# CederGroupHub/chgnet

Hardware: AMD Instinct MI355X
Metric: structures/s (energy+force+stress) on batched ~50-atom crystals (higher is better)
Workload: dtype f32

## Files before the change

### chgnet_amd/_lib.py

```python

from __future__ import annotations

import ctypes
import os

c_int_p = ctypes.POINTER(ctypes.c_int32)
c_float_p = ctypes.POINTER(ctypes.c_float)

TASK_BITS = {"e": 1, "f": 2, "s": 4, "m": 8}

EXPORTED_SYMBOLS = (
    "chg_abi_version", "chg_device_count", "chg_weights_required", "chg_engine_create", "chg_engine_destroy", "chg_last_error",
    "chg_batch_upload", "chg_batch_build", "chg_batch_build_predict", "chg_debug_fetch_i32", "chg_batch_update_geometry", "chg_batch_free", "chg_batch_device_bytes",
    "chg_predict", "chg_synchronize", "chg_batch_download", "chg_timer_start", "chg_timer_stop_ms",
    "chg_profile_enable", "chg_profile_reset", "chg_profile_count", "chg_profile_read",
    "chg_debug_fetch", "chg_test_rows_gemm", "chg_test_split_gemm",
    "chg_engine_set_memory_limit", "chg_engine_memory_info", "chg_batch_bytes_required",
    "chg_stream_copy", "chg_backward", "chg_engine_build_stats", "chg_engine_update_weights",
    "chg_engine_set_graph_search", "chg_engine_cell_stats",
    "chg_comm_unique_id", "chg_comm_create", "chg_comm_all_gather_f32", "chg_comm_all_reduce_sum_f32", "chg_comm_barrier",
    "chg_comm_destroy", "chg_comm_last_error",
    "chg_comm_all_gather_f32_device", "chg_comm_all_reduce_sum_f32_device", "chg_comm_reserve", "chg_comm_info",
    "chg_backward_allreduce", "chg_batch_all_gather_energy", "chg_engine_stream", "chg_engine_device",
    "chg_host_alloc", "chg_host_free",
    "chg_relax_create", "chg_relax_run", "chg_relax_download", "chg_relax_free", "chg_test_relax_step",
    "chg_md_create", "chg_md_run", "chg_md_download", "chg_md_free", "chg_test_md_step",
)


class ModelDesc(ctypes.Structure):
    _fields_ = [
        ("n_conv", ctypes.c_int32), ("cutoff_coeff", ctypes.c_int32), ("is_intensive", ctypes.c_int32),
        ("has_composition", ctypes.c_int32), ("atom_graph_cutoff", ctypes.c_float),
        ("bond_graph_cutoff", ctypes.c_float), ("n_weights", ctypes.c_int64),
        ("n_mlp_hidden", ctypes.c_int32), ("mlp_out_bias", ctypes.c_int32),
    ]


class BatchHost(ctypes.Structure):
# ... 118 lines not shown
    lib.chg_batch_update_geometry.argtypes = [vp, vp, c_float_p, c_float_p]
    lib.chg_batch_free.argtypes = [vp, vp]
    lib.chg_batch_device_bytes.argtypes = [vp]
    lib.chg_batch_device_bytes.restype = ctypes.c_int64
    lib.chg_predict.argtypes = [vp, vp, ctypes.c_uint32]
    lib.chg_synchronize.argtypes = [vp]
    lib.chg_backward.argtypes = [vp, vp, c_float_p, c_float_p, c_float_p, c_float_p, c_float_p]
    lib.chg_backward_allreduce.argtypes = [vp, vp, c_float_p, c_float_p, c_float_p, c_float_p, vp, c_float_p]
    lib.chg_batch_all_gather_energy.argtypes = [vp, vp, vp, ctypes.c_int64, c_float_p]
    lib.chg_engine_stream.argtypes = [vp]
    lib.chg_engine_stream.restype = ctypes.c_void_p
    lib.chg_engine_device.argtypes = [vp]
    lib.chg_engine_update_weights.argtypes = [vp, c_float_p]
    lib.chg_batch_download.argtypes = [vp, vp, ctypes.POINTER(OutHost)]
    lib.chg_timer_start.argtypes = [vp]
    lib.chg_timer_stop_ms.argtypes = [vp, c_float_p]
    lib.chg_stream_copy.argtypes = [vp, ctypes.c_int64, ctypes.c_int, c_float_p]
    lib.chg_profile_enable.argtypes = [vp, ctypes.c_int]
    lib.chg_profile_reset.argtypes = [vp]
    lib.chg_profile_count.argtypes = [vp]
    lib.chg_profile_read.argtypes = [vp, ctypes.c_int, ctypes.c_char_p, ctypes.c_int, ctypes.POINTER(ctypes.c_int64), ctypes.POINTER(ctypes.c_double)]
    lib.chg_debug_fetch.argtypes = [vp, vp, ctypes.c_char_p, c_float_p, ctypes.c_int64, ctypes.POINTER(ctypes.c_int64)]
    lib.chg_test_rows_gemm.argtypes = [vp, c_float_p, c_float_p, c_float_p, c_float_p, ctypes.c_int, ctypes.c_int, ctypes.c_int]
    lib.chg_test_split_gemm.argtypes = [vp, c_float_p, c_float_p, c_float_p, ctypes.c_int, ctypes.c_int, ctypes.c_int]
    dp = ctypes.POINTER(ctypes.c_double)
    lib.chg_relax_create.argtypes = [vp, ctypes.POINTER(StructsHost), ctypes.POINTER(RelaxParams), ctypes.POINTER(vp)]
    lib.chg_relax_run.argtypes = [vp, vp, ctypes.c_int32, c_int_p]
    lib.chg_relax_download.argtypes = [vp, vp, ctypes.POINTER(RelaxOutHost)]
    lib.chg_relax_free.argtypes = [vp, vp]
    lib.chg_test_relax_step.argtypes = [vp, ctypes.POINTER(RelaxParams), ctypes.c_int32, c_int_p, dp, dp, dp, c_int_p, c_float_p, c_float_p,
                                        c_float_p, c_float_p, dp, dp]
    lib.chg_md_create.argtypes = [vp, ctypes.POINTER(StructsHost), dp, dp, ctypes.POINTER(MdParams), ctypes.POINTER(vp)]
    lib.chg_md_run.argtypes = [vp, vp, ctypes.c_int32]
    lib.chg_md_download.argtypes = [vp, vp, ctypes.POINTER(MdOutHost)]
    lib.chg_md_free.argtypes = [vp, vp]
    lib.chg_test_md_step.argtypes = [vp, ctypes.POINTER(MdParams), ctypes.c_int32, c_int_p, ctypes.c_int32, dp, dp, dp, dp, dp, c_int_p,
                                     c_float_p, c_float_p, c_float_p, dp, dp]
    for name in EXPORTED_SYMBOLS:
        fn = getattr(lib, name)
        if fn.restype is ctypes.c_int and name not in ("chg_device_count", "chg_profile_count"):
            fn.restype = ctypes.c_int
    _LIB = lib
    return lib


def task_mask(task: str) -> int:
# ... 5 lines not shown
```

### chgnet_amd/csrc/engine.hip

```cpp

#include "engine_internal.h"
#include <cstring>

namespace chgh {

template <int UNROLL>
__global__ __launch_bounds__(256) void k_stream_copy(const f32x4* __restrict__ src, f32x4* __restrict__ dst, size_t n) {
  const size_t stride = (size_t)gridDim.x * blockDim.x;
  size_t i = (size_t)blockIdx.x * blockDim.x + threadIdx.x;
  for (; i + (UNROLL - 1) * stride < n; i += UNROLL * stride) {
    f32x4 v[UNROLL];
#pragma unroll
    for (int u = 0; u < UNROLL; ++u) v[u] = __builtin_nontemporal_load(src + i + u * stride);
#pragma unroll
    for (int u = 0; u < UNROLL; ++u) __builtin_nontemporal_store(v[u], dst + i + u * stride);
  }
  for (; i < n; i += stride) dst[i] = src[i];
}

template <bool NT>
__global__ __launch_bounds__(256) void k_stream_copy_seg(const f32x4* __restrict__ src, f32x4* __restrict__ dst, size_t n) {
  constexpr size_t SEG = 1024;
  const size_t nseg = n / SEG;
  for (size_t sgm = blockIdx.x; sgm < nseg; sgm += gridDim.x) {
// ... 526 lines not shown
  hipFree(a); hipFree(b);
  *ms_per_iter = best;
  return s;
}

int chg_test_rows_gemm(chg_engine* eng, const float* x, const float* wt, const float* bias, float* y, int rows, int k, int nout) {
  if (!eng || !x || !wt || !y || rows <= 0) return CHG_EINVAL;
  HIP_TRY(eng, hipSetDevice(eng->device));
  float *dx = nullptr, *dw = nullptr, *db = nullptr, *dy = nullptr;
  HIP_TRY(eng, hipMalloc(&dx, sizeof(float) * (size_t)rows * k));
  HIP_TRY(eng, hipMalloc(&dw, sizeof(float) * (size_t)nout * k));
  HIP_TRY(eng, hipMalloc(&db, sizeof(float) * (size_t)nout));
  HIP_TRY(eng, hipMalloc(&dy, sizeof(float) * (size_t)rows * nout));
  HIP_TRY(eng, hipMemcpy(dx, x, sizeof(float) * (size_t)rows * k, hipMemcpyHostToDevice));
  HIP_TRY(eng, hipMemcpy(dw, wt, sizeof(float) * (size_t)nout * k, hipMemcpyHostToDevice));
  if (bias) HIP_TRY(eng, hipMemcpy(db, bias, sizeof(float) * (size_t)nout, hipMemcpyHostToDevice));
  int s = rows_gemm(eng, "test_gemm", k, nout, dx, k, nullptr, dw, bias ? db : nullptr, nullptr, 0, dy, nout, nullptr, rows, 0);
  if (s == CHG_OK && hipStreamSynchronize(eng->stream) != hipSuccess) { eng->err = "test gemm failed"; s = CHG_EHIP; }
  if (s == CHG_OK) hipMemcpy(y, dy, sizeof(float) * (size_t)rows * nout, hipMemcpyDeviceToHost);
  hipFree(dx); hipFree(dw); hipFree(db); hipFree(dy);
  return s;
}

int chg_test_split_gemm(chg_engine* eng, const float* x, const float* w, float* y, int rows, int f, int mode) {
  if (!eng || !x || !w || !y || rows <= 0 || (f != D && f != 2 * D) || mode < 0 || mode > 3) return CHG_EINVAL;
  HIP_TRY(eng, hipSetDevice(eng->device));
  const int kin = (mode & 1) ? f : D, nout = (mode & 1) ? D : f;
  float *dx = nullptr, *dw = nullptr, *dy = nullptr;
  HIP_TRY(eng, hipMalloc(&dx, sizeof(float) * (size_t)rows * kin));
  HIP_TRY(eng, hipMalloc(&dw, sizeof(float) * (size_t)f * D));
  HIP_TRY(eng, hipMalloc(&dy, sizeof(float) * (size_t)rows * nout));
  HIP_TRY(eng, hipMemcpy(dx, x, sizeof(float) * (size_t)rows * kin, hipMemcpyHostToDevice));
  HIP_TRY(eng, hipMemcpy(dw, w, sizeof(float) * (size_t)f * D, hipMemcpyHostToDevice));
  hipStream_t st = eng->stream;
  switch (mode * 2 + (f == D ? 0 : 1)) {
    case 0: launch_test_split<0, D>(st, dx, dw, dy, rows); break;
    case 1: launch_test_split<0, 2 * D>(st, dx, dw, dy, rows); break;
    case 2: launch_test_split<1, D>(st, dx, dw, dy, rows); break;
    case 3: launch_test_split<1, 2 * D>(st, dx, dw, dy, rows); break;
    case 4: launch_test_split<2, D>(st, dx, dw, dy, rows); break;
    case 5: launch_test_split<2, 2 * D>(st, dx, dw, dy, rows); break;
    case 6: launch_test_split<3, D>(st, dx, dw, dy, rows); break;
    default: launch_test_split<3, 2 * D>(st, dx, dw, dy, rows); break;
  }
  int s = CHG_OK;
  if (hipGetLastError() != hipSuccess || hipStreamSynchronize(st) != hipSuccess) { eng->err = "chg_test_split_gemm failed"; s = CHG_EHIP; }
// ... 7 lines not shown
```

### chgnet_amd/csrc/engine_internal.h

```cpp
#pragma once

#include "chgnet_hip.h"

#include <hip/hip_runtime.h>

#include <algorithm>
#include <cmath>
#include <cstdint>
#include <cstdio>
#include <cstdlib>
#include <cstring>
#include <functional>
#include <map>
#include <mutex>
#include <string>
#include <unordered_map>
#include <vector>

#include "mfma_tile.h"
#include "mfma_split.h"
#include "kernels_conv.h"
#include "kernels_angle_w.h"
#include "kernels_angle_blk.h"
#include "kernels_embed.h"
// ... 221 lines not shown
template <class T>
int d2h(chg_engine* eng, T* dst, const T* src, size_t n) {
  if (n == 0 || !dst) return CHG_OK;
  HIP_TRY(eng, hipMemcpyAsync(dst, src, n * sizeof(T), hipMemcpyDeviceToHost, eng->stream));
  return CHG_OK;
}

template <class K>
int set_lds(chg_engine* eng, K kernel, size_t bytes) {
  HIP_TRY(eng, hipFuncSetAttribute(reinterpret_cast<const void*>(kernel), hipFuncAttributeMaxDynamicSharedMemorySize, (int)bytes));
  return CHG_OK;
}

size_t layout_weights(const float* base, int L, Weights& w);
int grid_for(int rows, int max_blocks, int block_rows = BLOCK_ROWS);
int tile_grid(chg_engine* eng, int rows, int block_rows = BLOCK_ROWS);
int rows_gemm(chg_engine* eng, const char* label, int K, int NOUT, const float* X, int ldx, const int* in_idx, const float* Wt,
              const float* bias, const float* resid, int ldr, float* Y, int ldy, const int* out_idx, int rows, int accumulate);
int rows_gemm_out2(chg_engine* eng, const char* label, const float* X, const int* in_idx, const float* Wt, const float* Wt2,
                   const float* bias, float* Y, int ldy, int rows);
int rows_gemm_in2(chg_engine* eng, const char* label, const float* X, int ldx, const float* Wt, const float* Wt2, float* Y,
                  const int* out_idx, int rows, int accumulate);
int zero(chg_engine* eng, void* p, size_t bytes);
int build_images(chg_engine* eng);
int predict_set_lds(chg_engine* eng);
int atomconv_q_table(chg_engine* eng, chg_batch* b, int l);
AtomConvArgs atomconv_args(chg_engine* eng, chg_batch* b, int l);
AngleArgs angle_args(chg_batch* b, int slot, const float* ang, const float* w_ang, const GatedW& g, float* out);
int angle_table_grads(chg_engine* eng, chg_batch* b, int slot, const float* w_bij_t, const float* w_ctr_t);
BondEmbedTArgs bond_embed_args(chg_engine* eng, chg_batch* b);
AngleEmbedTArgs angle_embed_args(chg_engine* eng, chg_batch* b);
int run_predict(chg_engine* eng, chg_batch* b, uint32_t task);
void carve(chg_batch* b, char* base, size_t& total);
int prepare_windows(chg_engine* eng, chg_batch* b);
inline long team_min_angles() {
  static const long v = [] { const char* e = std::getenv("CHGNET_TEAM_MIN_ANGLES"); return e ? std::atol(e) : 131072L; }();
  return v;
}
inline long blk_max_angles() {
  static const long v = [] { const char* e = std::getenv("CHGNET_BLK_MAX_ANGLES"); return e ? std::atol(e) : (1L << 22); }();
  return v;
}
inline size_t blk_tile_bound(size_t A, size_t Eb, size_t N) { return (A + 14 * Eb + 9 * N) / 16 + 1; }
inline int upload_blk_cap(size_t N, size_t A, size_t Eb) {
  return (A > 0 && N + 1 <= 8192 && (long)A <= blk_max_angles()) ? (int)blk_tile_bound(A, Eb, N) : 0;
}
// ... 28 lines not shown
```

### chgnet_amd/csrc/engine_predict.hip

```cpp
#include "engine_internal.h"

#include "kernels_geom.h"
#include "kernels_angle_fa.h"
#include "kernels_chain.h"

namespace chgh {


struct Cursor {
  const float* base;
  size_t pos = 0;
  const float* take(size_t n) {
    pos += (4 - pos % 4) % 4;
    const float* p = base + pos;
    pos += n;
    return p;
  }
};

void take_gated_tail(Cursor& c, GatedW& g, const float*& w2c_t, const float*& w2g_t) {
  g.w2c = c.take(D * D); g.b2c = c.take(D); g.w2g = c.take(D * D); g.b2g = c.take(D);
  w2c_t = c.take(D * D); w2g_t = c.take(D * D);
}
void take_ln(Cursor& c, GatedW& g) {
// ... 509 lines not shown
  a.ang0 = b->ang[0]; a.Gang = b->Gang; a.Gu = b->Gu;
  return a;
}

static int embed_grid_mult() {
  static const int m = [] { const char* e = std::getenv("CHGNET_EMBED_GRID_MULT"); return e ? std::atoi(e) : 2; }();
  return m;
}

struct ChainBuilder {
  ChainArgs a{};
  int max_rows = 0;
  ChainProb& add(int rows) {
    ChainProb& p = a.p[a.n++];
    p = ChainProb{};
    p.rows = rows;
    max_rows = std::max(max_rows, rows);
    return p;
  }
  static void term(ChainProb& p, const float* X, int ldx, const int* idx, const float* W, int K) { p.t[p.nterms++] = ChainTerm{X, idx, W, ldx, K}; }
  static void out(ChainProb& p, const float* W, const float* bias, float* Y, int ldy, int ncols) { p.o[p.nouts++] = ChainOut{W, bias, Y, ldy, ncols}; }
};
int launch_chain(chg_engine* eng, const char* label, ChainBuilder& cb) {
  int blocks = 0;
  for (int i = 0; i < cb.a.n; ++i) {
    ChainProb& p = cb.a.p[i];
    p.col_blocks = 0;
    for (int o = 0; o < p.nouts; ++o) p.col_blocks += p.o[o].ncols / D;
    p.serial_outs = (p.Y1 && p.Y1 == p.add) ? 1 : 0;
    if (p.serial_outs) {
      if (p.nouts > 1 || (p.nouts == 1 && p.o[0].ncols != D)) { eng->err = "launch_chain: an in-place problem takes one 64-column output"; return CHG_EINVAL; }
      p.col_blocks = 1;
    }
    p.col_blocks = std::max(1, p.col_blocks);
    blocks += p.col_blocks;
  }
  if (cb.max_rows <= 0 || blocks == 0) return CHG_OK;
  int row_blocks = 1;
  for (int i = 0; i < cb.a.n; ++i) {
    const int rows_per_wg = chain_tiles_per_wg(cb.a.p[i].nterms) * TILE_ROWS;
    row_blocks = std::max(row_blocks, (cb.a.p[i].rows + rows_per_wg - 1) / rows_per_wg);
  }
  LaunchScope ls(eng, label);
  hipLaunchKernelGGL(k_rows_chain, dim3(row_blocks, blocks), dim3(BLOCK), chain_lds(), eng->stream, cb.a);
  HIP_TRY(eng, hipGetLastError());
  return CHG_OK;
}

int forward_tiny(chg_engine* eng, chg_batch* b, bool want_grad, bool want_m) {
  const Weights& w = eng->w;
  const int L = b->L;
  for (int l = 0; l < L - 1; ++l) {
    TRY(atomconv_fwd_kernel(eng, b, l, want_grad));
    {
      ChainBuilder cb;
      ChainProb& p = cb.add(b->N);
      cb.term(p, b->agg_l[l], D, nullptr, w.ac[l].w_out, D);
      p.bias1 = w.ac[l].b_out; p.add = b->atom[l]; p.lda = D; p.Y1 = b->atom[l + 1]; p.ldy1 = D;
      cb.out(p, w.bc[l].w_ctr, w.bc[l].b1, b->Sl[l], 2 * D, 2 * D);
      cb.out(p, w.ac[l + 1].w_cn, w.ac[l + 1].b1, b->Pl[l + 1], 4 * D, 2 * D);
      cb.out(p, w.ac[l + 1].w_cn + 2 * D * D, nullptr, b->Pl[l + 1] + 2 * D, 4 * D, 2 * D);
      if (l < L - 2) cb.out(p, w.au[l].w_ctr, w.au[l].b1, b->Sl[L + l], 2 * D, 2 * D);
      if (l == 0) {
        ChainProb& q = cb.add(b->Eb);
        q.add = b->hbc[0]; q.lda = D;
        cb.out(q, w.bc[0].w_bij, nullptr, b->Rl[0], 4 * D, 2 * D);
        cb.out(q, w.bc[0].w_bij + 2 * D * D, nullptr, b->Rl[0] + 2 * D, 4 * D, 2 * D);
      }
      TRY(launch_chain(eng, "chain_A", cb));
// ... 105 lines not shown
      LaunchScope ls(eng, "embed_fwd");
      hipLaunchKernelGGL(k_embed_all<false>, dim3(ea.g_bond1 + ea.g_bond2 + ea.g_angle), dim3(BLOCK), bond_embed_lds(), st, ea);
    } else { LaunchScope ls(eng, "bond_embed_fwd");
      static const int o4 = [] { const char* e = std::getenv("CHGNET_EMBED_O4"); return e ? std::atoi(e) : 1; }();
      if (o4) hipLaunchKernelGGL((k_bond_embed_fwd_o4<1>), dim3(grid_for(b->Eu, o4 * 2 * eng->num_cus)), dim3(BLOCK), bond_embed_lds(), st, bond_embed_args(eng, b));
      else
      hipLaunchKernelGGL((k_bond_embed_t<false, false, 1>), dim3(grid_for(b->Eu, 2 * eng->num_cus)), dim3(BLOCK), bond_embed_lds(), st, bond_embed_args(eng, b));
      if (b->Eb > 0)
        hipLaunchKernelGGL((k_bond_embed_t<false, false, 2>), dim3(grid_for(b->Eb, 2 * eng->num_cus)), dim3(BLOCK), bond_embed_lds(), st, bond_embed_args(eng, b)); }
  }
  if (b->A > 0 && !(tiny && b->Ed > 0)) {
    LaunchScope ls(eng, "angle_embed_fwd");
    static const int o4 = [] { const char* e = std::getenv("CHGNET_EMBED_O4"); return e ? std::atoi(e) : 1; }();
    if (o4) hipLaunchKernelGGL((k_angle_embed_fwd_o4<0>), dim3(grid_for(b->A, o4 * embed_grid_mult() * eng->num_cus)), dim3(BLOCK), angle_embed_lds(), st, angle_embed_args(eng, b));
    else
    hipLaunchKernelGGL((k_angle_embed_t<false>), dim3(grid_for(b->A, embed_grid_mult() * eng->num_cus)), dim3(BLOCK), angle_embed_lds(), st, angle_embed_args(eng, b));
  }
  if (!tiny) { LaunchScope ls(eng, "atom_embed");
    hipLaunchKernelGGL(k_atom_embed, g1((int64_t)b->N * (D / 4)), dim3(256), 0, st, b->z, w.emb, b->atom[0], b->N); }
  HIP_TRY(eng, hipGetLastError());

  if (!tiny) TRY(zero(eng, b->zero1, zero_bytes));
  static const bool chain_on = [] { const char* e = std::getenv("CHGNET_TINY_CHAIN"); return !e || std::atoi(e) != 0; }();
  const bool chained = tiny && chain_on && fuse_gq() && L >= 2 && b->Ed > 0 && b->A > 0 && b->Eb > 0 && b->p_table_done == 0;
  if (chained) {
    TRY(forward_tiny(eng, b, want_grad, want_m));
  } else {
  for (int l = 0; l < L - 1; ++l) {
    TRY(atomconv_fwd(eng, b, l, want_grad));
    if (b->A > 0) {
      TRY(bondconv_fwd(eng, b, l));
      if (l < L - 2) TRY(angleupd_fwd(eng, b, l));
    }
  }
  if (want_m) {
    LaunchScope ls(eng, "magmom");
    hipLaunchKernelGGL(k_magmom, dim3(wave_grid(eng, b->N)), dim3(256), 0, st, b->atom[L - 1], w.site_w, w.site_b, b->magmom, b->N);
  }
  TRY(atomconv_fwd(eng, b, L - 1, want_grad));
  }

  {
    ReadoutArgs r{};
    r.atom = b->atom[L]; r.atom_owner = b->atom_owner; r.z = b->z; r.n_atoms = b->N;
    r.ln_g = w.ro_ln_g; r.ln_b = w.ro_ln_b; r.w0 = w.mlp_w0; r.b0 = w.mlp_b0; r.w1 = w.mlp_w1; r.b1 = w.mlp_b1;
    r.w2 = w.mlp_w2; r.b2 = w.mlp_b2; r.w3 = w.mlp_w3; r.b3 = w.mlp_b3; r.atomref = w.atomref;
    r.has_composition = eng->desc.has_composition; r.n_hidden = eng->desc.n_mlp_hidden;
    r.site_energy = b->site_energy; r.site_raw = b->site_raw; r.crystal_fea = b->crystal_fea;
// ... 256 lines not shown
  if ((s = set_lds(eng, k_angle_bwd_w<false>, angle_w_lds<false>()))) return s;
  if ((s = set_lds(eng, (k_angle_bwd_w<true, true>), angle_w_lds<true>()))) return s;
  if ((s = set_lds(eng, (k_angle_bwd_w<true, false, true>), angle_w_lds<true>()))) return s;
  if ((s = set_lds(eng, (k_angle_bwd_w<true, true, true>), angle_w_lds<true>()))) return s;
  if ((s = set_lds(eng, (k_angle_bwd_w<false, true>), angle_w_lds<false>()))) return s;
  if ((s = set_lds(eng, k_angle<true, false>, angle_lds<true>()))) return s;
  if ((s = set_lds(eng, k_angle<true, true>, (angle_lds<true, WAVES, true>())))) return s;
  if ((s = set_lds(eng, k_angle<false, true>, (angle_lds<false, WAVES, true>())))) return s;
  if ((s = set_lds(eng, k_angle<false, false, FWD_WAVES>, (angle_lds<false, FWD_WAVES>())))) return s;
#ifdef CHG_EXPERIMENTS
  if ((s = set_lds(eng, (k_angle<true, false, 4>), (size_t)100 << 10))) return s;
  if ((s = set_lds(eng, (k_angle<false, false, 4>), (size_t)100 << 10))) return s;
  if ((s = set_lds(eng, k_atomconv_fwd<4>, (size_t)100 << 10))) return s;
#endif
  if ((s = set_lds(eng, k_readout<false>, readout_lds()))) return s;
  if ((s = set_lds(eng, (k_bond_embed_t<false, false, 1>), bond_embed_lds()))) return s;
  if ((s = set_lds(eng, (k_bond_embed_t<false, false, 2>), bond_embed_lds()))) return s;
  if ((s = set_lds(eng, (k_bond_embed_t<true, false, 1>), bond_embed_lds()))) return s;
  if ((s = set_lds(eng, (k_bond_embed_t<true, false, 2>), bond_embed_lds()))) return s;
  if ((s = set_lds(eng, k_angle_embed_t<false>, angle_embed_lds()))) return s;
  if ((s = set_lds(eng, k_angle_embed_fwd_o4<0>, angle_embed_lds()))) return s;
  if ((s = set_lds(eng, k_bond_embed_fwd_o4<1>, bond_embed_lds()))) return s;
  if ((s = set_lds(eng, k_angle_embed_t<true>, angle_embed_lds()))) return s;
  if ((s = set_lds(eng, k_rows_chain, chain_lds()))) return s;
  if ((s = set_lds(eng, k_embed_all<false>, bond_embed_lds()))) return s;
  if ((s = set_lds(eng, k_embed_all<true>, bond_embed_lds()))) return s;
  return CHG_OK;
}


}
```

### chgnet_amd/csrc/kernels_chain.h

```cpp
#pragma once

#include "kernels_conv.h"

namespace chg {

constexpr int CHAIN_TERMS = 3, CHAIN_OUTS = 4, CHAIN_PROBS = 2;
struct ChainTerm {
  const float* X;
  const int* idx;
  const float* W;
  int ldx, K;
};
struct ChainOut {
  const float* W;
  const float* bias;
  float* Y;
  int ldy, ncols;
};
struct ChainProb {
  int rows, nterms, nouts, col_blocks;
  int serial_outs;
  ChainTerm t[CHAIN_TERMS];
  const float* bias1;
  const float* add;
  const int* add_idx;
  int lda;
  float* Y1;
  const int* y1_idx;
  int ldy1;
  ChainOut o[CHAIN_OUTS];
};
struct ChainArgs {
  ChainProb p[CHAIN_PROBS];
  int n;
};

__host__ __device__ constexpr int chain_tiles_per_wg(int nterms) { return nterms >= 2 ? 4 : WAVES; }
constexpr int CH_TS = D + PAD;
constexpr int CH_W1 = D * (2 * D + PAD);
constexpr size_t chain_lds() {
  return sizeof(float) * ((size_t)CHAIN_TERMS * CH_W1 + (size_t)D * (D + PAD) + D + D + (size_t)WAVES * TILE_ROWS * CH_TS);
}

struct ChainW { f32x4 v[4]; };
struct ChainX { f32x4 v[8]; };
__device__ __forceinline__ void chain_ws_issue(ChainW& r, const float* __restrict__ W, int K, int tid) {
  const int nchunks = (K / 32) * 4 * D;
#pragma unroll
  for (int q = 0; q < 2; ++q) {
    const int c = tid + q * BLOCK;
    if (c < nchunks) {
      const int f = c % D, g = (c / D) & 3, mk = c / (4 * D);
      const float* src = W + (size_t)f * K + 32 * mk + 4 * g;
      r.v[2 * q] = *reinterpret_cast<const f32x4*>(src);
      r.v[2 * q + 1] = *reinterpret_cast<const f32x4*>(src + 16);
    }
  }
}
__device__ __forceinline__ void chain_ws_commit(const ChainW& r, h16x8* img, int K, int tid) {
  const int nchunks = (K / 32) * 4 * D;
#pragma unroll
  for (int q = 0; q < 2; ++q) {
    const int c = tid + q * BLOCK;
    if (c < nchunks) {
      h16x8 hi, lo;
// ... 14 lines not shown
  }
}
template <int K>
__device__ __forceinline__ void chain_x_contract(f32x4 (&acc)[VT], const ChainX& r, const float* W1, float* T, int lane, int j, int g) {
  constexpr int LPR = K / 4, RPS = 64 / LPR, NV = TILE_ROWS / RPS, KT = K / 16;
  const int sub = lane / LPR, t = lane % LPR;
  f32x4 x[KT];
#pragma unroll
  for (int h = 0; h < K / D; ++h) {
    if ((t >> 4) == h) {
#pragma unroll
      for (int it = 0; it < NV; ++it) *reinterpret_cast<f32x4*>(T + (RPS * it + sub) * CH_TS + 4 * (t & 15)) = r.v[it];
    }
    __builtin_amdgcn_wave_barrier();
    f32x4 xh[VT];
    read_dl<VT>(T + j * CH_TS, g, xh);
#pragma unroll
    for (int f = 0; f < VT; ++f) x[VT * h + f] = xh[f];
    __builtin_amdgcn_wave_barrier();
  }
  gemm_split<KT, VT, true>(acc, reinterpret_cast<const h16x8*>(W1), D, x, j, g);
}

static __global__ __launch_bounds__(BLOCK) CHG_TWO_WAVES void k_rows_chain(ChainArgs a) {
  extern __shared__ __attribute__((aligned(16))) float smem[];
  float* W1 = smem;
  float* W2 = W1 + CHAIN_TERMS * CH_W1;
  float* b1s = W2 + D * (D + PAD);
  float* b2s = b1s + D;
  float* tiles = b2s + D;
  int y = blockIdx.y, pi = 0;
  for (; pi < a.n; ++pi) {
    if (y < a.p[pi].col_blocks) break;
    y -= a.p[pi].col_blocks;
  }
  if (pi >= a.n) return;
  const ChainProb& p = a.p[pi];
  const int cb = y;
  const int tpw = chain_tiles_per_wg(p.nterms);
  if ((int)blockIdx.x * tpw * TILE_ROWS >= p.rows) return;
  const int tid = threadIdx.x, wave = tid >> 6, lane = tid & 63, j = lane & 15, g = lane >> 4;
  const int row0 = (blockIdx.x * tpw + wave) * TILE_ROWS;
  const int nvalid = wave < tpw ? min(TILE_ROWS, p.rows - row0) : 0;
  const bool active = nvalid > 0;
  const int rr_ = active ? row0 + min(j, nvalid - 1) : 0;
  float* T = tiles + wave * TILE_ROWS * CH_TS;
  int in_row[CHAIN_TERMS];
#pragma unroll
  for (int t = 0; t < CHAIN_TERMS; ++t) in_row[t] = (t < p.nterms && p.t[t].idx) ? p.t[t].idx[rr_] : rr_;
  const int add_row = (p.add && p.add_idx) ? p.add_idx[rr_] : rr_;
  const int y1_row = (p.Y1 && p.y1_idx) ? p.y1_idx[rr_] : rr_;
  ChainW wr[CHAIN_TERMS], w2r;
#pragma unroll
  for (int t = 0; t < CHAIN_TERMS; ++t)
    if (t < p.nterms) chain_ws_issue(wr[t], p.t[t].W, p.t[t].K, tid);
  int lb = cb, oi = 0;
  for (; oi < p.nouts - 1; ++oi) {
    const int nb = p.o[oi].ncols >> 6;
    if (lb < nb) break;
    lb -= nb;
  }
  if (p.nouts) chain_ws_issue(w2r, p.o[oi].W + (size_t)lb * D * D, D, tid);
  float bias1 = 0.f, bias2 = 0.f;
  if (tid < D && p.bias1) bias1 = p.bias1[tid];
  if (p.nouts && tid < D && p.o[oi].bias) bias2 = p.o[oi].bias[lb * D + tid];
  ChainX xr[CHAIN_TERMS];
  const int sub4 = lane >> 4, t4 = lane & 15;
  f32x4 av[TILE_ROWS / 4];
  int orow[TILE_ROWS / 4];
  if (active) {
#pragma unroll
    for (int t = 0; t < CHAIN_TERMS; ++t)
      if (t < p.nterms) {
        if (p.t[t].K == D) chain_x_issue<D>(xr[t], p.t[t], in_row[t], lane);
        else chain_x_issue<2 * D>(xr[t], p.t[t], in_row[t], lane);
      }
#pragma unroll
    for (int it = 0; it < TILE_ROWS / 4; ++it) {
      const int rr = 4 * it + sub4;
      const int ra = __shfl(add_row, rr);
      orow[it] = __shfl(y1_row, rr);
      av[it] = zero4();
      if (p.add) av[it] = *reinterpret_cast<const f32x4*>(p.add + (size_t)ra * p.lda + 4 * t4);
    }
  }
  if (tid < D) { b1s[tid] = bias1; b2s[tid] = bias2; }
  if (p.nouts) chain_ws_commit(w2r, reinterpret_cast<h16x8*>(W2), D, tid);
#pragma unroll
  for (int t = 0; t < CHAIN_TERMS; ++t)
    if (t < p.nterms) chain_ws_commit(wr[t], reinterpret_cast<h16x8*>(W1 + t * CH_W1), p.t[t].K, tid);
  __syncthreads();
  if (!active) return;
  f32x4 acc[VT];
  read_dl<VT>(b1s, g, acc);
#pragma unroll
  for (int t = 0; t < CHAIN_TERMS; ++t)
    if (t < p.nterms) {
      if (p.t[t].K == D) chain_x_contract<D>(acc, xr[t], W1 + t * CH_W1, T, lane, j, g);
      else chain_x_contract<2 * D>(acc, xr[t], W1 + t * CH_W1, T, lane, j, g);
    }
  write_dl<VT>(T + j * CH_TS, g, acc);
  __builtin_amdgcn_wave_barrier();
#pragma unroll
  for (int it = 0; it < TILE_ROWS / 4; ++it) {
    av[it] += *reinterpret_cast<const f32x4*>(T + (4 * it + sub4) * CH_TS + 4 * t4);
    asm volatile("" : "+v"(av[it]));
  }
#pragma unroll
  for (int it = 0; it < TILE_ROWS / 4; ++it) {
    const int rr = 4 * it + sub4;
    *reinterpret_cast<f32x4*>(T + rr * CH_TS + 4 * t4) = av[it];
    if (p.Y1 && cb == 0 && rr < nvalid) *reinterpret_cast<f32x4*>(p.Y1 + (size_t)orow[it] * p.ldy1 + 4 * t4) = av[it];
  }
  if (p.nouts == 0) return;
  __builtin_amdgcn_wave_barrier();
  f32x4 x2[VT];
  read_dl<VT>(T + j * CH_TS, g, x2);
  __builtin_amdgcn_wave_barrier();
  const ChainOut& o = p.o[oi];
  f32x4 acc2[VT];
  read_dl<VT>(b2s, g, acc2);
  gemm_split<VT, VT, true>(acc2, reinterpret_cast<const h16x8*>(W2), D, x2, j, g);
  write_dl<VT>(T + j * CH_TS, g, acc2);
  __builtin_amdgcn_wave_barrier();
#pragma unroll
  for (int it = 0; it < TILE_ROWS / 4; ++it) {
    const int rr = 4 * it + sub4;
    if (rr < nvalid)
      *reinterpret_cast<f32x4*>(o.Y + (size_t)(row0 + rr) * o.ldy + lb * D + 4 * t4) = *reinterpret_cast<const f32x4*>(T + rr * CH_TS + 4 * t4);
  }
}

}
```

### chgnet_amd/engine.py

```python

from __future__ import annotations

import ctypes
import weakref

import numpy as np

from chgnet_amd import _lib
from chgnet_amd.graph.structure import atomic_numbers_of
from chgnet_amd.pack import D, PackedBatch, PackedWeights, _check_z, pack_batch


def _fp(a: np.ndarray):
    return a.ctypes.data_as(_lib.c_float_p)


def _ip(a: np.ndarray):
    return a.ctypes.data_as(_lib.c_int_p)


class PreparedStructures:

    __slots__ = ("n_struct", "z", "atom_off", "frac", "lattice")

# ... 291 lines not shown
            n, ms = ctypes.c_int64(), ctypes.c_double()
            self._check(self.lib.chg_profile_read(self.handle, i, buf, 64, ctypes.byref(n), ctypes.byref(ms)))
            out[buf.value.decode()] = (int(n.value), float(ms.value))
        return out

    def debug_fetch(self, batch: DeviceBatch, name: str, shape) -> np.ndarray:
        n = int(np.prod(shape))
        dst = np.empty(max(n, 1), np.float32)
        got = ctypes.c_int64()
        self._check(self.lib.chg_debug_fetch(self.handle, batch.handle, name.encode(), _fp(dst), n, ctypes.byref(got)))
        if got.value != n:
            raise RuntimeError(f"debug_fetch({name}): expected {n} floats, device buffer has {got.value}")
        return dst[:n].reshape(shape)

    def test_split_gemm(self, x: np.ndarray, w: np.ndarray, mode: int) -> np.ndarray:
        x = np.ascontiguousarray(x, np.float32)
        w = np.ascontiguousarray(w, np.float32)
        f = w.shape[0]
        assert w.shape[1] == 64 and x.shape[1] == (f if mode & 1 else 64)
        y = np.empty((x.shape[0], 64 if mode & 1 else f), np.float32)
        self._check(self.lib.chg_test_split_gemm(self.handle, _fp(x), _fp(w), _fp(y), x.shape[0], f, int(mode)))
        return y

    def test_rows_gemm(self, x: np.ndarray, wt: np.ndarray, bias: np.ndarray | None) -> np.ndarray:
        x = np.ascontiguousarray(x, np.float32)
        wt = np.ascontiguousarray(wt, np.float32)
        rows, k = x.shape
        nout = wt.shape[0]
        y = np.empty((rows, nout), np.float32)
        b = np.ascontiguousarray(bias, np.float32) if bias is not None else None
        self._check(self.lib.chg_test_rows_gemm(self.handle, _fp(x), _fp(wt), _fp(b) if b is not None else None, _fp(y), rows, k, nout))
        return y
```

### include/chgnet_hip.h

```cpp
#ifndef CHGNET_HIP_H
#define CHGNET_HIP_H

#include <stdint.h>

#ifdef __cplusplus
extern "C" {
#endif

typedef enum {
  CHG_OK = 0,
  CHG_EINVAL = -1,
  CHG_EHIP = -2,
  CHG_ENOMEM = -3,
  CHG_ENODEV = -4,
  CHG_EUNSUPPORTED = -5,
  CHG_ERANGE = -6
} chg_status;

enum {
  CHG_TASK_E = 1u,
  CHG_TASK_F = 2u,
  CHG_TASK_S = 4u,
  CHG_TASK_M = 8u
};
// ... 90 lines not shown
                 const float* force_cotangent, const float* stress_cotangent, float* grad_blob);
struct chg_comm;
int chg_backward_allreduce(chg_engine* eng, chg_batch* batch, const float* energy_cotangent, const float* magmom_cotangent,
                           const float* force_cotangent, const float* stress_cotangent, struct chg_comm* comm, float* grad_blob);
int chg_batch_all_gather_energy(chg_engine* eng, chg_batch* batch, struct chg_comm* comm, int64_t width, float* table);
void* chg_engine_stream(chg_engine* eng);
int chg_engine_device(chg_engine* eng);
int chg_engine_update_weights(chg_engine* eng, const float* weights_blob);
int chg_batch_download(chg_engine* eng, chg_batch* batch, const chg_out_host* out);

int chg_timer_start(chg_engine* eng);
int chg_timer_stop_ms(chg_engine* eng, float* elapsed_ms);

int chg_stream_copy(chg_engine* eng, int64_t bytes, int iters, float* ms_per_iter);

int chg_profile_enable(chg_engine* eng, int on);
int chg_profile_reset(chg_engine* eng);
int chg_profile_count(chg_engine* eng);
int chg_profile_read(chg_engine* eng, int i, char* label, int label_cap, int64_t* launches, double* total_ms);

int chg_debug_fetch(chg_engine* eng, chg_batch* batch, const char* name, float* dst, int64_t capacity, int64_t* n_written);

int chg_test_rows_gemm(chg_engine* eng, const float* x, const float* wt, const float* bias, float* y, int rows, int k, int nout);
int chg_test_split_gemm(chg_engine* eng, const float* x, const float* w, float* y, int rows, int f, int mode);

enum { CHG_RELAX_RUNNING = 0, CHG_RELAX_CONVERGED = 1, CHG_RELAX_MAX_STEPS = 2, CHG_RELAX_NONFINITE = 3 };
typedef struct chg_relax_params {
  double fmax;
  int32_t max_steps, relax_cell;
  double dt, maxstep, dtmax, finc, fdec, astart, fa;
  int32_t nmin;
  double exp_cell_factor;
  double r_atom, r_bond, numerical_tol;
  double stress_weight;
} chg_relax_params;
typedef struct chg_relax chg_relax;
typedef struct chg_relax_out_host {
  double* frac;
  double* lattice;
  float* energy;
  float* force;
  float* stress;
  float* magmom;
  int32_t* n_steps;
  int32_t* status;
} chg_relax_out_host;
// ... 72 lines not shown
```

Before: 38540.

## Make row-chain kernel persistent with multi-column weight staging and enable for all batches

The fused row-chain kernel becomes persistent: when the one-shot grid would exceed the CU count, each workgroup loops over row blocks and keeps several output-column weight blocks in LDS, reusing staged weights instead of reloading them per block. The kernel is templated on term count so LDS is sized to the actual number of terms, and the next tile's loads are issued early to overlap with compute. The chained forward path is no longer limited to tiny batches, so larger batches now take it as well. This risks lower occupancy from larger LDS use and less parallelism on big batches. A test entry point for the chain kernel is added.

```diff
diff --git a/chgnet_amd/_lib.py b/chgnet_amd/_lib.py
--- a/chgnet_amd/_lib.py
+++ b/chgnet_amd/_lib.py
@@ -14,7 +14,7 @@
     "chg_batch_upload", "chg_batch_build", "chg_batch_build_predict", "chg_debug_fetch_i32", "chg_batch_update_geometry", "chg_batch_free", "chg_batch_device_bytes",
     "chg_predict", "chg_synchronize", "chg_batch_download", "chg_timer_start", "chg_timer_stop_ms",
     "chg_profile_enable", "chg_profile_reset", "chg_profile_count", "chg_profile_read",
-    "chg_debug_fetch", "chg_test_rows_gemm", "chg_test_split_gemm",
+    "chg_debug_fetch", "chg_test_rows_gemm", "chg_test_rows_chain", "chg_test_split_gemm",
     "chg_engine_set_memory_limit", "chg_engine_memory_info", "chg_batch_bytes_required",
     "chg_stream_copy", "chg_backward", "chg_engine_build_stats", "chg_engine_update_weights",
     "chg_engine_set_graph_search", "chg_engine_cell_stats",
@@ -179,6 +179,7 @@
     lib.chg_profile_read.argtypes = [vp, ctypes.c_int, ctypes.c_char_p, ctypes.c_int, ctypes.POINTER(ctypes.c_int64), ctypes.POINTER(ctypes.c_double)]
     lib.chg_debug_fetch.argtypes = [vp, vp, ctypes.c_char_p, c_float_p, ctypes.c_int64, ctypes.POINTER(ctypes.c_int64)]
     lib.chg_test_rows_gemm.argtypes = [vp, c_float_p, c_float_p, c_float_p, c_float_p, ctypes.c_int, ctypes.c_int, ctypes.c_int]
+    lib.chg_test_rows_chain.argtypes = [vp, c_float_p, c_float_p, c_float_p, c_int_p, c_float_p, c_float_p, ctypes.c_int, ctypes.c_int]
     lib.chg_test_split_gemm.argtypes = [vp, c_float_p, c_float_p, c_float_p, ctypes.c_int, ctypes.c_int, ctypes.c_int]
     dp = ctypes.POINTER(ctypes.c_double)
     lib.chg_relax_create.argtypes = [vp, ctypes.POINTER(StructsHost), ctypes.POINTER(RelaxParams), ctypes.POINTER(vp)]
diff --git a/chgnet_amd/csrc/engine.hip b/chgnet_amd/csrc/engine.hip
--- a/chgnet_amd/csrc/engine.hip
+++ b/chgnet_amd/csrc/engine.hip
@@ -572,6 +572,34 @@
   return s;
 }
 
+int chg_test_rows_chain(chg_engine* eng, const float* x, const float* w, float* g, const int* idx, const float* wout, float* y, int rows, int n_g) {
+  if (!eng || !x || !w || !g || !idx || !wout || !y || rows <= 0 || n_g <= 0) return CHG_EINVAL;
+  for (int r = 0; r < rows; ++r)
+    if (idx[r] < 0 || idx[r] >= n_g) return CHG_EINVAL;
+  HIP_TRY(eng, hipSetDevice(eng->device));
+  float *dx = nullptr, *dw = nullptr, *dg = nullptr, *dwo = nullptr, *dy = nullptr;
+  int* di = nullptr;
+  HIP_TRY(eng, hipMalloc(&dx, sizeof(float) * (size_t)rows * 4 * D));
+  HIP_TRY(eng, hipMalloc(&dw, sizeof(float) * 4 * D * D));
+  HIP_TRY(eng, hipMalloc(&dg, sizeof(float) * (size_t)n_g * D));
+  HIP_TRY(eng, hipMalloc(&di, sizeof(int) * (size_t)rows));
+  HIP_TRY(eng, hipMalloc(&dwo, sizeof(float) * D * D));
+  HIP_TRY(eng, hipMalloc(&dy, sizeof(float) * (size_t)rows * D));
+  HIP_TRY(eng, hipMemcpy(dx, x, sizeof(float) * (size_t)rows * 4 * D, hipMemcpyHostToDevice));
+  HIP_TRY(eng, hipMemcpy(dw, w, sizeof(float) * 4 * D * D, hipMemcpyHostToDevice));
+  HIP_TRY(eng, hipMemcpy(dg, g, sizeof(float) * (size_t)n_g * D, hipMemcpyHostToDevice));
+  HIP_TRY(eng, hipMemcpy(di, idx, sizeof(int) * (size_t)rows, hipMemcpyHostToDevice));
+  HIP_TRY(eng, hipMemcpy(dwo, wout, sizeof(float) * D * D, hipMemcpyHostToDevice));
+  int s = test_rows_chain(eng, dx, dw, dg, di, dwo, dy, rows);
+  if (s == CHG_OK && hipStreamSynchronize(eng->stream) != hipSuccess) { eng->err = "test chain failed"; s = CHG_EHIP; }
+  if (s == CHG_OK) {
+    hipMemcpy(g, dg, sizeof(float) * (size_t)n_g * D, hipMemcpyDeviceToHost);
+    hipMemcpy(y, dy, sizeof(float) * (size_t)rows * D, hipMemcpyDeviceToHost);
+  }
+  hipFree(dx); hipFree(dw); hipFree(dg); hipFree(di); hipFree(dwo); hipFree(dy);
+  return s;
+}
+
 int chg_test_split_gemm(chg_engine* eng, const float* x, const float* w, float* y, int rows, int f, int mode) {
   if (!eng || !x || !w || !y || rows <= 0 || (f != D && f != 2 * D) || mode < 0 || mode > 3) return CHG_EINVAL;
   HIP_TRY(eng, hipSetDevice(eng->device));
diff --git a/chgnet_amd/csrc/engine_internal.h b/chgnet_amd/csrc/engine_internal.h
--- a/chgnet_amd/csrc/engine_internal.h
+++ b/chgnet_amd/csrc/engine_internal.h
@@ -267,6 +267,7 @@
 int rows_gemm_in2(chg_engine* eng, const char* label, const float* X, int ldx, const float* Wt, const float* Wt2, float* Y,
                   const int* out_idx, int rows, int accumulate);
 int zero(chg_engine* eng, void* p, size_t bytes);
+int test_rows_chain(chg_engine* eng, const float* X, const float* W, float* G, const int* idx, const float* Wout, float* Y, int rows);
 int build_images(chg_engine* eng);
 int predict_set_lds(chg_engine* eng);
 int atomconv_q_table(chg_engine* eng, chg_batch* b, int l);
diff --git a/chgnet_amd/csrc/engine_predict.hip b/chgnet_amd/csrc/engine_predict.hip
--- a/chgnet_amd/csrc/engine_predict.hip
+++ b/chgnet_amd/csrc/engine_predict.hip
@@ -555,29 +555,70 @@
   static void out(ChainProb& p, const float* W, const float* bias, float* Y, int ldy, int ncols) { p.o[p.nouts++] = ChainOut{W, bias, Y, ldy, ncols}; }
 };
 int launch_chain(chg_engine* eng, const char* label, ChainBuilder& cb) {
-  int blocks = 0;
-  for (int i = 0; i < cb.a.n; ++i) {
-    ChainProb& p = cb.a.p[i];
+  ChainArgs& A = cb.a;
+  A.nt1 = 1;
+  int one_shot_wgs = 0, max_row_blocks = 1;
+  for (int i = 0; i < A.n; ++i) {
+    ChainProb& p = A.p[i];
+    A.nt1 = std::max(A.nt1, p.nterms);
     p.col_blocks = 0;
     for (int o = 0; o < p.nouts; ++o) p.col_blocks += p.o[o].ncols / D;
     p.serial_outs = (p.Y1 && p.Y1 == p.add) ? 1 : 0;
-    if (p.serial_outs) {
-      if (p.nouts > 1 || (p.nouts == 1 && p.o[0].ncols != D)) { eng->err = "launch_chain: an in-place problem takes one 64-column output"; return CHG_EINVAL; }
-      p.col_blocks = 1;
+    if (p.serial_outs && (p.nouts > 1 || (p.nouts == 1 && p.o[0].ncols != D))) {
+      eng->err = "launch_chain: an in-place problem takes one 64-column output";
+      return CHG_EINVAL;
     }
     p.col_blocks = std::max(1, p.col_blocks);
-    blocks += p.col_blocks;
-  }
-  if (cb.max_rows <= 0 || blocks == 0) return CHG_OK;
-  int row_blocks = 1;
-  for (int i = 0; i < cb.a.n; ++i) {
-    const int rows_per_wg = chain_tiles_per_wg(cb.a.p[i].nterms) * TILE_ROWS;
-    row_blocks = std::max(row_blocks, (cb.a.p[i].rows + rows_per_wg - 1) / rows_per_wg);
+    p.tpw = chain_tiles_per_wg(p.nterms);
+    p.cpw = 1;
+    const int rows_per_wg = p.tpw * TILE_ROWS;
+    const int row_blocks = (p.rows + rows_per_wg - 1) / rows_per_wg;
+    max_row_blocks = std::max(max_row_blocks, row_blocks);
+    one_shot_wgs += row_blocks * p.col_blocks;
+  }
+  if (cb.max_rows <= 0) return CHG_OK;
+  int gx = max_row_blocks, gy = 0, cpw_max = 1;
+  if (one_shot_wgs <= eng->num_cus) {
+    for (int i = 0; i < A.n; ++i) { A.p[i].wgs = gx; gy += A.p[i].col_blocks; }
+  } else {
+    const size_t fixed = chain_lds_floats(A.nt1, 0), cap = chain_lds() / sizeof(float);
+    const int fit = std::max(1, (int)((cap - fixed) / (CH_W2 + D)));
+    long work = 0;
+    int rbs[CHAIN_PROBS];
+    for (int i = 0; i < A.n; ++i) {
+      ChainProb& p = A.p[i];
+      p.tpw = WAVES;
+      const int groups = (p.col_blocks + fit - 1) / fit;
+      p.cpw = (p.col_blocks + groups - 1) / groups;
+      p.col_blocks = groups;
+      cpw_max = std::max(cpw_max, p.cpw);
+      rbs[i] = (p.rows + WAVES * TILE_ROWS - 1) / (WAVES * TILE_ROWS);
+      work += (long)rbs[i] * groups;
+    }
+    gx = 1;
+    for (int i = 0; i < A.n; ++i) {
+      ChainProb& p = A.p[i];
+      p.wgs = (int)std::max<long>(1, std::min<long>(rbs[i], (long)eng->num_cus * rbs[i] / std::max<long>(1, work)));
+      gx = std::max(gx, p.wgs);
+      gy += p.col_blocks;
+    }
   }
   LaunchScope ls(eng, label);
-  hipLaunchKernelGGL(k_rows_chain, dim3(row_blocks, blocks), dim3(BLOCK), chain_lds(), eng->stream, cb.a);
+  const size_t lds = sizeof(float) * chain_lds_floats(A.nt1, cpw_max);
+  if (A.nt1 == 1) hipLaunchKernelGGL(k_rows_chain<1>, dim3(gx, gy), dim3(BLOCK), lds, eng->stream, A);
+  else hipLaunchKernelGGL(k_rows_chain<CHAIN_TERMS>, dim3(gx, gy), dim3(BLOCK), lds, eng->stream, A);
   HIP_TRY(eng, hipGetLastError());
   return CHG_OK;
+}
+
+int test_rows_chain(chg_engine* eng, const float* X, const float* W, float* G, const int* idx, const float* Wout, float* Y, int rows) {
+  ChainBuilder cb;
+  ChainProb& p = cb.add(rows);
+  cb.term(p, X, 4 * D, nullptr, W, 2 * D);
+  cb.term(p, X + 2 * D, 4 * D, nullptr, W + 2 * D * D, 2 * D);
+  p.add = G; p.add_idx = idx; p.lda = D; p.Y1 = G; p.y1_idx = idx; p.ldy1 = D;
+  cb.out(p, Wout, nullptr, Y, D, D);
+  return launch_chain(eng, "test_chain", cb);
 }
 
 int forward_tiny(chg_engine* eng, chg_batch* b, bool want_grad, bool want_m) {
@@ -729,8 +770,9 @@
 
   if (!tiny) TRY(zero(eng, b->zero1, zero_bytes));
   static const bool chain_on = [] { const char* e = std::getenv("CHGNET_TINY_CHAIN"); return !e || std::atoi(e) != 0; }();
-  const bool chained = tiny && chain_on && fuse_gq() && L >= 2 && b->Ed > 0 && b->A > 0 && b->Eb > 0 && b->p_table_done == 0;
+  const bool chained = chain_on && fuse_gq() && L >= 2 && b->Ed > 0 && b->A > 0 && b->Eb > 0;
   if (chained) {
+    TRY(atomconv_tables(eng, b, 0));
     TRY(forward_tiny(eng, b, want_grad, want_m));
   } else {
   for (int l = 0; l < L - 1; ++l) {
@@ -1033,7 +1075,8 @@
   if ((s = set_lds(eng, k_angle_embed_fwd_o4<0>, angle_embed_lds()))) return s;
   if ((s = set_lds(eng, k_bond_embed_fwd_o4<1>, bond_embed_lds()))) return s;
   if ((s = set_lds(eng, k_angle_embed_t<true>, angle_embed_lds()))) return s;
-  if ((s = set_lds(eng, k_rows_chain, chain_lds()))) return s;
+  if ((s = set_lds(eng, k_rows_chain<1>, chain_lds()))) return s;
+  if ((s = set_lds(eng, k_rows_chain<CHAIN_TERMS>, chain_lds()))) return s;
   if ((s = set_lds(eng, k_embed_all<false>, bond_embed_lds()))) return s;
   if ((s = set_lds(eng, k_embed_all<true>, bond_embed_lds()))) return s;
   return CHG_OK;
diff --git a/chgnet_amd/csrc/kernels_chain.h b/chgnet_amd/csrc/kernels_chain.h
--- a/chgnet_amd/csrc/kernels_chain.h
+++ b/chgnet_amd/csrc/kernels_chain.h
@@ -20,6 +20,9 @@
 struct ChainProb {
   int rows, nterms, nouts, col_blocks;
   int serial_outs;
+  int tpw;
+  int cpw;
+  int wgs;
   ChainTerm t[CHAIN_TERMS];
   const float* bias1;
   const float* add;
@@ -33,14 +36,17 @@
 struct ChainArgs {
   ChainProb p[CHAIN_PROBS];
   int n;
+  int nt1;
 };
 
 __host__ __device__ constexpr int chain_tiles_per_wg(int nterms) { return nterms >= 2 ? 4 : WAVES; }
 constexpr int CH_TS = D + PAD;
 constexpr int CH_W1 = D * (2 * D + PAD);
-constexpr size_t chain_lds() {
-  return sizeof(float) * ((size_t)CHAIN_TERMS * CH_W1 + (size_t)D * (D + PAD) + D + D + (size_t)WAVES * TILE_ROWS * CH_TS);
-}
+constexpr int CH_W2 = D * (D + PAD);
+__host__ __device__ constexpr size_t chain_lds_floats(int nt1, int cpw) {
+  return (size_t)nt1 * CH_W1 + (size_t)cpw * (CH_W2 + D) + D + (size_t)WAVES * TILE_ROWS * CH_TS;
+}
+constexpr size_t chain_lds() { return sizeof(float) * chain_lds_floats(CHAIN_TERMS, 1); }
 
 struct ChainW { f32x4 v[4]; };
 struct ChainX { f32x4 v[8]; };
@@ -101,13 +107,49 @@
   gemm_split<KT, VT, true>(acc, reinterpret_cast<const h16x8*>(W1), D, x, j, g);
 }
 
-static __global__ __launch_bounds__(BLOCK) CHG_TWO_WAVES void k_rows_chain(ChainArgs a) {
+__device__ __forceinline__ void chain_block(const ChainProb& p, int gb, int& oi, int& lb) {
+  lb = gb; oi = 0;
+  for (; oi < p.nouts - 1; ++oi) {
+    const int nb = p.o[oi].ncols >> 6;
+    if (lb < nb) break;
+    lb -= nb;
+  }
+}
+
+template <int NT>
+struct ChainTile {
+  ChainX xr[NT];
+  f32x4 av[TILE_ROWS / 4];
+  int orow[TILE_ROWS / 4];
+};
+template <int NT>
+__device__ __forceinline__ void chain_tile_issue(ChainTile<NT>& c, const ChainProb& p, int row0, int nvalid, int lane) {
+  const int j = lane & 15, sub4 = lane >> 4, t4 = lane & 15;
+  const int rr_ = row0 + min(j, nvalid - 1);
+  int in_row[NT];
+#pragma unroll
+  for (int t = 0; t < NT; ++t) in_row[t] = (t < p.nterms && p.t[t].idx) ? p.t[t].idx[rr_] : rr_;
+  const int add_row = (p.add && p.add_idx) ? p.add_idx[rr_] : rr_;
+  const int y1_row = (p.Y1 && p.y1_idx) ? p.y1_idx[rr_] : rr_;
+#pragma unroll
+  for (int t = 0; t < NT; ++t)
+    if (t < p.nterms) {
+      if (p.t[t].K == D) chain_x_issue<D>(c.xr[t], p.t[t], in_row[t], lane);
+      else chain_x_issue<2 * D>(c.xr[t], p.t[t], in_row[t], lane);
+    }
+#pragma unroll
+  for (int it = 0; it < TILE_ROWS / 4; ++it) {
+    const int rr = 4 * it + sub4;
+    const int ra = __shfl(add_row, rr);
+    c.orow[it] = __shfl(y1_row, rr);
+    c.av[it] = zero4();
+    if (p.add) c.av[it] = *reinterpret_cast<const f32x4*>(p.add + (size_t)ra * p.lda + 4 * t4);
+  }
+}
+
+template <int NT>
+__global__ __launch_bounds__(BLOCK) CHG_TWO_WAVES void k_rows_chain(ChainArgs a) {
   extern __shared__ __attribute__((aligned(16))) float smem[];
-  float* W1 = smem;
-  float* W2 = W1 + CHAIN_TERMS * CH_W1;
-  float* b1s = W2 + D * (D + PAD);
-  float* b2s = b1s + D;
-  float* tiles = b2s + D;
   int y = blockIdx.y, pi = 0;
   for (; pi < a.n; ++pi) {
     if (y < a.p[pi].col_blocks) break;
@@ -115,99 +157,104 @@
   }
   if (pi >= a.n) return;
   const ChainProb& p = a.p[pi];
-  const int cb = y;
-  const int tpw = chain_tiles_per_wg(p.nterms);
-  if ((int)blockIdx.x * tpw * TILE_ROWS >= p.rows) return;
+  const int cg = y;
+  const int tpw = p.tpw;
+  if ((int)blockIdx.x >= p.wgs || (int)blockIdx.x * tpw * TILE_ROWS >= p.rows) return;
+  float* W1 = smem;
+  float* W2 = W1 + a.nt1 * CH_W1;
+  float* b2s = W2 + p.cpw * CH_W2;
+  float* b1s = b2s + p.cpw * D;
+  float* tiles = b1s + D;
   const int tid = threadIdx.x, wave = tid >> 6, lane = tid & 63, j = lane & 15, g = lane >> 4;
-  const int row0 = (blockIdx.x * tpw + wave) * TILE_ROWS;
-  const int nvalid = wave < tpw ? min(TILE_ROWS, p.rows - row0) : 0;
-  const bool active = nvalid > 0;
-  const int rr_ = active ? row0 + min(j, nvalid - 1) : 0;
+  const int sub4 = lane >> 4, t4 = lane & 15;
   float* T = tiles + wave * TILE_ROWS * CH_TS;
-  int in_row[CHAIN_TERMS];
-#pragma unroll
-  for (int t = 0; t < CHAIN_TERMS; ++t) in_row[t] = (t < p.nterms && p.t[t].idx) ? p.t[t].idx[rr_] : rr_;
-  const int add_row = (p.add && p.add_idx) ? p.add_idx[rr_] : rr_;
-  const int y1_row = (p.Y1 && p.y1_idx) ? p.y1_idx[rr_] : rr_;
-  ChainW wr[CHAIN_TERMS], w2r;
-#pragma unroll
-  for (int t = 0; t < CHAIN_TERMS; ++t)
+  int tot_blocks = 0;
+  for (int o = 0; o < p.nouts; ++o) tot_blocks += p.o[o].ncols >> 6;
+  const int blk0 = cg * p.cpw, nb = max(0, min(p.cpw, tot_blocks - blk0));
+  int rb = blockIdx.x;
+  int row0 = (rb * tpw + wave) * TILE_ROWS;
+  int nvalid = wave < tpw ? min(TILE_ROWS, p.rows - row0) : 0;
+  ChainW wr[NT], w2r;
+#pragma unroll
+  for (int t = 0; t < NT; ++t)
     if (t < p.nterms) chain_ws_issue(wr[t], p.t[t].W, p.t[t].K, tid);
-  int lb = cb, oi = 0;
-  for (; oi < p.nouts - 1; ++oi) {
-    const int nb = p.o[oi].ncols >> 6;
-    if (lb < nb) break;
-    lb -= nb;
-  }
-  if (p.nouts) chain_ws_issue(w2r, p.o[oi].W + (size_t)lb * D * D, D, tid);
+  int oi = 0, lb = 0;
+  if (nb) {
+    chain_block(p, blk0, oi, lb);
+    chain_ws_issue(w2r, p.o[oi].W + (size_t)lb * D * D, D, tid);
+  }
   float bias1 = 0.f, bias2 = 0.f;
   if (tid < D && p.bias1) bias1 = p.bias1[tid];
-  if (p.nouts && tid < D && p.o[oi].bias) bias2 = p.o[oi].bias[lb * D + tid];
-  ChainX xr[CHAIN_TERMS];
-  const int sub4 = lane >> 4, t4 = lane & 15;
-  f32x4 av[TILE_ROWS / 4];
-  int orow[TILE_ROWS / 4];
-  if (active) {
-#pragma unroll
-    for (int t = 0; t < CHAIN_TERMS; ++t)
+  if (nb && tid < D && p.o[oi].bias) bias2 = p.o[oi].bias[lb * D + tid];
+  ChainTile<NT> c;
+  if (nvalid > 0) chain_tile_issue(c, p, row0, nvalid, lane);
+  if (tid < D) { b1s[tid] = bias1; b2s[tid] = bias2; }
+  if (nb) chain_ws_commit(w2r, reinterpret_cast<h16x8*>(W2), D, tid);
+#pragma unroll
+  for (int t = 0; t < NT; ++t)
+    if (t < p.nterms) chain_ws_commit(wr[t], reinterpret_cast<h16x8*>(W1 + t * CH_W1), p.t[t].K, tid);
+  for (int k = 1; k < nb; ++k) {
+    chain_block(p, blk0 + k, oi, lb);
+    chain_ws_issue(w2r, p.o[oi].W + (size_t)lb * D * D, D, tid);
+    bias2 = (tid < D && p.o[oi].bias) ? p.o[oi].bias[lb * D + tid] : 0.f;
+    if (tid < D) b2s[k * D + tid] = bias2;
+    chain_ws_commit(w2r, reinterpret_cast<h16x8*>(W2 + k * CH_W2), D, tid);
+  }
+  __syncthreads();
+  while (nvalid > 0) {
+    f32x4 acc[VT];
+    read_dl<VT>(b1s, g, acc);
+#pragma unroll
+    for (int t = 0; t < NT; ++t)
       if (t < p.nterms) {
-        if (p.t[t].K == D) chain_x_issue<D>(xr[t], p.t[t], in_row[t], lane);
-        else chain_x_issue<2 * D>(xr[t], p.t[t], in_row[t], lane);
+        if (p.t[t].K == D) chain_x_contract<D>(acc, c.xr[t], W1 + t * CH_W1, T, lane, j, g);
+        else chain_x_contract<2 * D>(acc, c.xr[t], W1 + t * CH_W1, T, lane, j, g);
       }
+    write_dl<VT>(T + j * CH_TS, g, acc);
+    __builtin_amdgcn_wave_barrier();
+#pragma unroll
+    for (int it = 0; it < TILE_ROWS / 4; ++it) {
+      c.av[it] += *reinterpret_cast<const f32x4*>(T + (4 * it + sub4) * CH_TS + 4 * t4);
+      asm volatile("" : "+v"(c.av[it]));
+    }
 #pragma unroll
     for (int it = 0; it < TILE_ROWS / 4; ++it) {
       const int rr = 4 * it + sub4;
-      const int ra = __shfl(add_row, rr);
-      orow[it] = __shfl(y1_row, rr);
-      av[it] = zero4();
-      if (p.add) av[it] = *reinterpret_cast<const f32x4*>(p.add + (size_t)ra * p.lda + 4 * t4);
-    }
-  }
-  if (tid < D) { b1s[tid] = bias1; b2s[tid] = bias2; }
-  if (p.nouts) chain_ws_commit(w2r, reinterpret_cast<h16x8*>(W2), D, tid);
-#pragma unroll
-  for (int t = 0; t < CHAIN_TERMS; ++t)
-    if (t < p.nterms) chain_ws_commit(wr[t], reinterpret_cast<h16x8*>(W1 + t * CH_W1), p.t[t].K, tid);
-  __syncthreads();
-  if (!active) return;
-  f32x4 acc[VT];
-  read_dl<VT>(b1s, g, acc);
-#pragma unroll
-  for (int t = 0; t < CHAIN_TERMS; ++t)
-    if (t < p.nterms) {
-      if (p.t[t].K == D) chain_x_contract<D>(acc, xr[t], W1 + t * CH_W1, T, lane, j, g);
-      else chain_x_contract<2 * D>(acc, xr[t], W1 + t * CH_W1, T, lane, j, g);
-    }
-  write_dl<VT>(T + j * CH_TS, g, acc);
-  __builtin_amdgcn_wave_barrier();
-#pragma unroll
-  for (int it = 0; it < TILE_ROWS / 4; ++it) {
-    av[it] += *reinterpret_cast<const f32x4*>(T + (4 * it + sub4) * CH_TS + 4 * t4);
-    asm volatile("" : "+v"(av[it]));
-  }
-#pragma unroll
-  for (int it = 0; it < TILE_ROWS / 4; ++it) {
-    const int rr = 4 * it + sub4;
-    *reinterpret_cast<f32x4*>(T + rr * CH_TS + 4 * t4) = av[it];
-    if (p.Y1 && cb == 0 && rr < nvalid) *reinterpret_cast<f32x4*>(p.Y1 + (size_t)orow[it] * p.ldy1 + 4 * t4) = av[it];
-  }
-  if (p.nouts == 0) return;
-  __builtin_amdgcn_wave_barrier();
-  f32x4 x2[VT];
-  read_dl<VT>(T + j * CH_TS, g, x2);
-  __builtin_amdgcn_wave_barrier();
-  const ChainOut& o = p.o[oi];
-  f32x4 acc2[VT];
-  read_dl<VT>(b2s, g, acc2);
-  gemm_split<VT, VT, true>(acc2, reinterpret_cast<const h16x8*>(W2), D, x2, j, g);
-  write_dl<VT>(T + j * CH_TS, g, acc2);
-  __builtin_amdgcn_wave_barrier();
-#pragma unroll
-  for (int it = 0; it < TILE_ROWS / 4; ++it) {
-    const int rr = 4 * it + sub4;
-    if (rr < nvalid)
-      *reinterpret_cast<f32x4*>(o.Y + (size_t)(row0 + rr) * o.ldy + lb * D + 4 * t4) = *reinterpret_cast<const f32x4*>(T + rr * CH_TS + 4 * t4);
-  }
-}
-
-}
+      *reinterpret_cast<f32x4*>(T + rr * CH_TS + 4 * t4) = c.av[it];
+      if (p.Y1 && cg == 0 && rr < nvalid) *reinterpret_cast<f32x4*>(p.Y1 + (size_t)c.orow[it] * p.ldy1 + 4 * t4) = c.av[it];
+    }
+    const int cur0 = row0, cur_valid = nvalid;
+    rb += p.wgs;
+    row0 = (rb * tpw + wave) * TILE_ROWS;
+    nvalid = (wave < tpw && row0 < p.rows) ? min(TILE_ROWS, p.rows - row0) : 0;
+    if (nb == 0) {
+      __builtin_amdgcn_wave_barrier();
+      if (nvalid > 0) chain_tile_issue(c, p, row0, nvalid, lane);
+      continue;
+    }
+    __builtin_amdgcn_wave_barrier();
+    f32x4 x2[VT];
+    read_dl<VT>(T + j * CH_TS, g, x2);
+    __builtin_amdgcn_wave_barrier();
+    if (NT == 1 && nvalid > 0) chain_tile_issue(c, p, row0, nvalid, lane);
+    for (int k = 0; k < nb; ++k) {
+      chain_block(p, blk0 + k, oi, lb);
+      const ChainOut& o = p.o[oi];
+      f32x4 acc2[VT];
+      read_dl<VT>(b2s + k * D, g, acc2);
+      gemm_split<VT, VT, true>(acc2, reinterpret_cast<const h16x8*>(W2 + k * CH_W2), D, x2, j, g);
+      write_dl<VT>(T + j * CH_TS, g, acc2);
+      __builtin_amdgcn_wave_barrier();
+#pragma unroll
+      for (int it = 0; it < TILE_ROWS / 4; ++it) {
+        const int rr = 4 * it + sub4;
+        if (rr < cur_valid)
+          *reinterpret_cast<f32x4*>(o.Y + (size_t)(cur0 + rr) * o.ldy + lb * D + 4 * t4) = *reinterpret_cast<const f32x4*>(T + rr * CH_TS + 4 * t4);
+      }
+      __builtin_amdgcn_wave_barrier();
+    }
+    if (NT > 1 && nvalid > 0) chain_tile_issue(c, p, row0, nvalid, lane);
+  }
+}
+
+}
diff --git a/chgnet_amd/engine.py b/chgnet_amd/engine.py
--- a/chgnet_amd/engine.py
+++ b/chgnet_amd/engine.py
@@ -337,6 +337,19 @@
         self._check(self.lib.chg_test_split_gemm(self.handle, _fp(x), _fp(w), _fp(y), x.shape[0], f, int(mode)))
         return y
 
+    def test_rows_chain(self, x: np.ndarray, w: np.ndarray, g: np.ndarray, idx: np.ndarray, wout: np.ndarray) -> tuple[np.ndarray, np.ndarray]:
+        x = np.ascontiguousarray(x, np.float32)
+        w = np.ascontiguousarray(w, np.float32)
+        g = np.array(g, np.float32, order="C", copy=True)
+        idx = np.ascontiguousarray(idx, np.int32)
+        wout = np.ascontiguousarray(wout, np.float32)
+        rows = x.shape[0]
+        assert x.shape == (rows, 256) and w.shape == (2, 64, 128) and g.shape[1] == 64 and idx.shape == (rows,) and wout.shape == (64, 64)
+        y = np.empty((rows, 64), np.float32)
+        self._check(self.lib.chg_test_rows_chain(self.handle, _fp(x), _fp(w), _fp(g), idx.ctypes.data_as(ctypes.POINTER(ctypes.c_int32)),
+                                                 _fp(wout), _fp(y), rows, g.shape[0]))
+        return g, y
+
     def test_rows_gemm(self, x: np.ndarray, wt: np.ndarray, bias: np.ndarray | None) -> np.ndarray:
         x = np.ascontiguousarray(x, np.float32)
         wt = np.ascontiguousarray(wt, np.float32)
diff --git a/include/chgnet_hip.h b/include/chgnet_hip.h
--- a/include/chgnet_hip.h
+++ b/include/chgnet_hip.h
@@ -136,6 +136,7 @@
 int chg_debug_fetch(chg_engine* eng, chg_batch* batch, const char* name, float* dst, int64_t capacity, int64_t* n_written);
 
 int chg_test_rows_gemm(chg_engine* eng, const float* x, const float* wt, const float* bias, float* y, int rows, int k, int nout);
+int chg_test_rows_chain(chg_engine* eng, const float* x, const float* w, float* g, const int* idx, const float* wout, float* y, int rows, int n_g);
 int chg_test_split_gemm(chg_engine* eng, const float* x, const float* w, float* y, int rows, int f, int mode);
 
 enum { CHG_RELAX_RUNNING = 0, CHG_RELAX_CONVERGED = 1, CHG_RELAX_MAX_STEPS = 2, CHG_RELAX_NONFINITE = 3 };
```

New measurement: 38550, median of 6. Within noise of the previous version (+0.0%).
